# george-gca/sr-pytorch-lightning

Hardware: AMD Instinct MI355X
Metric: SR training throughput, LR patches/s (48x48 LR x4, fwd+bwd+Adam) (higher is better)
Workload: dtype bf16; 1 GPU; edsr_baseline x4, 48x48 LR patches, batch 256/GPU, train step (L1 + Adam); global_batch=256, parallelism=dp1, hip_graph=full

## Files before the change

sr-pytorch-lightning_amd/csrc/conv_lk.hip:

```cpp
#include <stdlib.h>
#include <type_traits>
#include "srk_common.h"

#ifndef SRK_LK5_STAMPS
#define SRK_LK5_STAMPS 0
#endif

namespace {

template <int DT, int CPP, int NRB, int K>
__global__ __launch_bounds__(256) void lk_conv_kernel(const srk_conv_args a, int tilesX, int tilesY, unsigned x_bytes, unsigned w_bytes) {
  typedef DTraits<DT> Tr;
  constexpr int PXB = CPP * 16;
  constexpr int ROWS = 32 * NRB;
  extern __shared__ __attribute__((aligned(16))) char smem[];
  constexpr int XT = 16 + K - 1, XTP = (XT + 1) & ~1;
  constexpr int xs_bytes = XT * XTP * PXB;
  constexpr int slab = K * CPP * ROWS * 16;
  char* const Xs = smem;
  char* const Wr = smem + ((xs_bytes + 1023) & ~1023);

  const int tid = threadIdx.x, lane = tid & 63;
  const int wave = __builtin_amdgcn_readfirstlane(tid >> 6);
  const int r = lane & 31, h = lane >> 5;
// ... 764 lines not shown
    {
      int n, y0, x0;
      tile_of(t, n, y0, x0);
#pragma unroll
      for (int pb = 0; pb < 2; ++pb) {
        const int gy = y0 + prow[pb], gx = x0 + px;
        const bool ok = h == 0 && gy < H && gx < W;
#pragma unroll
        for (int o = 0; o < 4; ++o) {
          if (o >= O) break;
#pragma unroll
          for (int i = 0; i < 2; ++i) {
            typedef __attribute__((ext_vector_type(2))) unsigned int u32x2_t;
            u32x2_t v;
            v.x = __float_as_uint(acc[pb][o * 4 + i * 2] * sc + pa[o]);
            v.y = __float_as_uint(acc[pb][o * 4 + i * 2 + 1] * sc + pa[o]);
            const unsigned off = ok ? (unsigned)((((n * O + o) * H2 + 2 * gy + i) * W2 + 2 * gx) * 4) : 0x80000000u;
            __builtin_amdgcn_raw_buffer_store_b64(v, orsrc, off, 0, SRK_AUX_WT);
          }
        }
      }
    }
  }
}

template <int DT, int NW>
__global__ __launch_bounds__(NW * 64) void lk5_rows_fwd_kernel(const srk_conv_args a, int nb, int segs, int seg_rows, int units, unsigned x_bytes) {
  typedef DTraits<DT> Tr;
  constexpr int AHEAD = NW == 4 ? 2 : 1, PRO = NW + 4 + (AHEAD - 1) * NW, RING = PRO + NW;
  constexpr int ROWB = 32 * 128, SP = 68, SCR = 32 * SP * 4;
  extern __shared__ __attribute__((aligned(16))) char smem[];
  const int tid = threadIdx.x, lane = tid & 63;
  const int wave = __builtin_amdgcn_readfirstlane(tid >> 6);
  const int r = lane & 31, h = lane >> 5;
  const int H = a.H, W = a.W, O = a.Cout >> 2;
  float* const scr = reinterpret_cast<float*>(smem + RING * ROWB + wave * SCR);
  const unsigned lds0 = lds_addr_of(smem);
  const __amdgpu_buffer_rsrc_t wrs = __builtin_amdgcn_make_buffer_rsrc(const_cast<void*>(a.wpk), 0, 25 * 8 * 32 * 16, 0x00020000);
  const i32x4 xrsrc = make_rsrc4(a.x, x_bytes);

  float bias6[6], pa3[3];
#pragma unroll
  for (int o = 0; o < 3; ++o) {
    pa3[o] = (a.post_add && o < O) ? a.post_add[o] : 0.f;
#pragma unroll
    for (int j = 0; j < 2; ++j) bias6[o * 2 + j] = (a.bias && o < O) ? a.bias[8 * o + h * 2 + j] : 0.f;
  }
  typedef __attribute__((ext_vector_type(4))) unsigned int u32x4_t;
  i32x4 A[5][4][2];
#pragma unroll
  for (int m = 0; m < 2; ++m) {
    const int R = m * 32 + r, kw = R / 12, co = R - kw * 12;
    const bool ok = R < 60 && co < a.Cout;
#pragma unroll
    for (int kh = 0; kh < 5; ++kh)
#pragma unroll
      for (int ks = 0; ks < 4; ++ks) {
        const unsigned off = ok ? (unsigned)(((((kh * 5 + kw) * 8 + 2 * ks + h) * 32 + 8 * (co >> 2) + (co & 3)) << 4)) : 0x80000000u;
        const u32x4_t v = __builtin_amdgcn_raw_buffer_load_b128(wrs, off, 0, 0);
        A[kh][ks][m] = i32x4{(int)v.x, (int)v.y, (int)v.z, (int)v.w};
      }
  }
  int ccol[4], cpx[4];
#pragma unroll
  for (int pc = 0; pc < 4; ++pc) {
    const int px = pc * 8 + (lane >> 3), sl = lane & 7, c = sl ^ swz(px);
    cpx[pc] = px - 2;
    ccol[pc] = ((px - 2) * a.x_pitch + a.x_coff + c * 8) * 2;
  }
  asm volatile("s_waitcnt vmcnt(0)" ::: "memory");

  const int bsw = swz(r);
  const int H2 = 2 * H, W2 = 2 * W;
  const float sc = a.scale;
  const __amdgpu_buffer_rsrc_t orsrc = __builtin_amdgcn_make_buffer_rsrc(a.out, 0, 0x7fffffff, 0x00020000);

  for (int u = blockIdx.x; u < units; u += gridDim.x) {
    const int sgm = u % segs, bb = (u / segs) % nb, n = u / (segs * nb);
    const int x0 = bb * 28, ys = sgm * seg_rows;
    const int ye = min(H, ys + seg_rows), nx = min(28, W - x0);
    const int steps = (ye - ys + NW - 1) / NW, qmax = (ye - ys) + 4;
    auto dma_row = [&](int q) {
      const int gy = ys - 2 + q;
      const bool rok = (unsigned)gy < (unsigned)H && q < qmax;
      const int base = ((n * H + gy) * W + x0) * a.x_pitch * 2;
      const unsigned dst = lds0 + (unsigned)((q % RING) * ROWB);
#pragma unroll
      for (int pc = 0; pc < 4; ++pc) {
        const bool ok = rok && (unsigned)(x0 + cpx[pc]) < (unsigned)W;
        dma16_hidden(xrsrc, ok ? (unsigned)(base + ccol[pc]) : 0x80000000u, (unsigned)__builtin_amdgcn_readfirstlane((int)(dst + pc * 1024)));
      }
    };
    asm volatile("s_waitcnt vmcnt(0) lgkmcnt(0)\n\ts_barrier" ::: "memory");
    for (int q = wave; q < PRO; q += NW) dma_row(q);

    f32x16 accp[2];
    int gyp = 0;
    auto epi_write = [&](int g0, int cnt) {
#pragma unroll
      for (int g = g0; g < g0 + cnt; ++g) {
        const int m = g >> 2, i = g & 3;
        *reinterpret_cast<f32x4*>(scr + r * SP + m * 32 + 8 * i + 4 * h) = f32x4{accp[m][4 * i], accp[m][4 * i + 1], accp[m][4 * i + 2], accp[m][4 * i + 3]};
      }
    };
    float ev[6];
    auto epi_read = [&](int t0, int cnt) {
#pragma unroll
      for (int t = t0; t < t0 + cnt; ++t) {
        const int o = t / 5, kw = t - o * 5;
        const f32x2 v = *reinterpret_cast<const f32x2*>(scr + (r + kw) * SP + kw * 12 + o * 4 + h * 2);
        ev[o * 2] = kw == 0 ? v.x : ev[o * 2] + v.x;
        ev[o * 2 + 1] = kw == 0 ? v.y : ev[o * 2 + 1] + v.y;
      }
    };
    auto epi_store = [&]() {
      const bool ok = r < nx && gyp < ye;
#pragma unroll
      for (int o = 0; o < 3; ++o) {
        typedef __attribute__((ext_vector_type(2))) unsigned int u32x2_t;
        u32x2_t v;
        v.x = __float_as_uint((ev[o * 2] + bias6[o * 2]) * sc + pa3[o]);
        v.y = __float_as_uint((ev[o * 2 + 1] + bias6[o * 2 + 1]) * sc + pa3[o]);
        const unsigned off = (ok && o < O) ? (unsigned)((((n * O + o) * H2 + 2 * gyp + h) * W2 + 2 * (x0 + r)) * 4) : 0x80000000u;
        __builtin_amdgcn_raw_buffer_store_b64(v, orsrc, off, 0, SRK_AUX_WT);
      }
    };
    auto step = [&](int s, auto epi_tag) {
      constexpr bool EPI = decltype(epi_tag)::value;
      if (!EPI) asm volatile("s_waitcnt vmcnt(0)" ::: "memory");
      else if (AHEAD == 1) { if (s == 1) asm volatile("s_waitcnt vmcnt(0)" ::: "memory"); else asm volatile("s_waitcnt vmcnt(3)" ::: "memory"); }
      else if (s == 1) asm volatile("s_waitcnt vmcnt(4)" ::: "memory");
      else if (s == 2) asm volatile("s_waitcnt vmcnt(7)" ::: "memory");
      else asm volatile("s_waitcnt vmcnt(10)" ::: "memory");
      asm volatile("s_waitcnt lgkmcnt(0)\n\ts_barrier" ::: "memory");
      dma_row(NW * s + PRO + wave);
      const int q0 = NW * s + wave;
      const char* rowp[5];
#pragma unroll
      for (int kh = 0; kh < 5; ++kh) rowp[kh] = smem + ((q0 + kh) % RING) * ROWB + r * 128;
      f32x16 acc[2];
#pragma unroll
      for (int e = 0; e < 16; ++e) { acc[0][e] = 0.f; acc[1][e] = 0.f; }
      constexpr int PF = 6;
      i32x4 bf[PF];
      auto bfrag = [&](int k) { return lds_read16(rowp[k >> 2] + (((2 * (k & 3) + h) ^ bsw) << 4)); };
#pragma unroll
      for (int k = 0; k < PF; ++k) bf[k] = bfrag(k);
#pragma unroll
      for (int k = 0; k < 20; ++k) {
        const i32x4 b = bf[k % PF];
        if (k + PF < 20) bf[k % PF] = bfrag(k + PF);
        if (EPI) {
          if (k < 8) epi_write(k, 1);
          else if (k == 8) asm volatile("" ::: "memory");
          else if (k >= 9 && k < 19) epi_read((k - 9) * 3 / 2, (k - 8) * 3 / 2 - (k - 9) * 3 / 2);
          else if (k == 19) epi_store();
        }
        acc[0] = Tr::mma(A[k >> 2][k & 3][0], b, acc[0]);
        acc[1] = Tr::mma(A[k >> 2][k & 3][1], b, acc[1]);
        __builtin_amdgcn_sched_barrier(0);
      }
      accp[0] = acc[0]; accp[1] = acc[1];
      gyp = ys + q0;
    };
    step(0, std::false_type{});
#pragma unroll 1
    for (int s = 1; s < steps; ++s) step(s, std::true_type{});
    epi_write(0, 8);
    asm volatile("" ::: "memory");
    epi_read(0, 15);
    epi_store();
  }
}

template <int DT>
__global__ __launch_bounds__(256) void lk5_dgrad_kernel(const srk_conv_args a, int nb, int segs, int seg_rows, int units, unsigned x_bytes) {
  typedef DTraits<DT> Tr;
  typedef typename Tr::elem elem;
  constexpr int RING = 16, ROWB = 36 * 32;
  extern __shared__ __attribute__((aligned(16))) char smem[];
  const int tid = threadIdx.x, lane = tid & 63;
  const int wave = __builtin_amdgcn_readfirstlane(tid >> 6);
  const int r = lane & 31, h = lane >> 5;
  const int H = a.H, W = a.W;
  const unsigned lds0 = lds_addr_of(smem);
  const __amdgpu_buffer_rsrc_t wrs = __builtin_amdgcn_make_buffer_rsrc(const_cast<void*>(a.wpk), 0, 25 * 2 * 64 * 16, 0x00020000);
  const i32x4 xrsrc = make_rsrc4(a.x, x_bytes);
  typedef __attribute__((ext_vector_type(4))) unsigned int u32x4_t;
  i32x4 A[25][2];
#pragma unroll
  for (int t = 0; t < 25; ++t)
#pragma unroll
    for (int m = 0; m < 2; ++m) {
      const u32x4_t v = __builtin_amdgcn_raw_buffer_load_b128(wrs, (unsigned)((((t * 2 + h) * 64 + m * 32 + r) << 4)), 0, 0);
      A[t][m] = i32x4{(int)v.x, (int)v.y, (int)v.z, (int)v.w};
    }
  const int c0 = ((lane >> 1) - 2) * a.x_pitch * 2 + (a.x_coff + (lane & 1) * 8) * 2, p0 = (lane >> 1) - 2;
  const int c1 = ((32 + (lane >> 1)) - 2) * a.x_pitch * 2 + (a.x_coff + (lane & 1) * 8) * 2, p1 = 32 + (lane >> 1) - 2;
  asm volatile("s_waitcnt vmcnt(0)" ::: "memory");

  const __amdgpu_buffer_rsrc_t orsrc = __builtin_amdgcn_make_buffer_rsrc(a.out, 0, 0x7fffffff, 0x00020000);
  for (int u = blockIdx.x; u < units; u += gridDim.x) {
    const int sgm = u % segs, bb = (u / segs) % nb, n = u / (segs * nb);
    const int x0 = bb * 32, ys = sgm * seg_rows;
    const int ye = min(H, ys + seg_rows);
    const int steps = (ye - ys + 3) >> 2, qmax = (ye - ys) + 4;
    auto dma_row = [&](int q) {
      const int gy = ys - 2 + q;
      const bool rok = (unsigned)gy < (unsigned)H && q < qmax;
      const int base = ((n * H + gy) * W + x0) * a.x_pitch * 2;
      const unsigned dst = lds0 + (unsigned)((q % RING) * ROWB);
      dma16_hidden(xrsrc, (rok && (unsigned)(x0 + p0) < (unsigned)W) ? (unsigned)(base + c0) : 0x80000000u, (unsigned)__builtin_amdgcn_readfirstlane((int)dst));
      if (lane < 8)
        dma16_hidden(xrsrc, (rok && (unsigned)(x0 + p1) < (unsigned)W) ? (unsigned)(base + c1) : 0x80000000u, (unsigned)__builtin_amdgcn_readfirstlane((int)(dst + 1024)));
    };
    asm volatile("s_waitcnt vmcnt(0) lgkmcnt(0)\n\ts_barrier" ::: "memory");
    dma_row(wave);
    dma_row(4 + wave);
    dma_row(8 + wave);
#if SRK_LK5_STAMPS
    unsigned long long* const stamp = (blockIdx.x == 0 && tid == 0 && u == blockIdx.x) ? reinterpret_cast<unsigned long long*>(const_cast<float*>(a.post_add)) : nullptr;
#define SRK_LSTAMP(i) do { if (stamp && s < 24) stamp[s * 8 + (i)] = __builtin_amdgcn_s_memtime(); } while (0)
#else
#define SRK_LSTAMP(i) do { } while (0)
#endif
    f32x16 accp[2];
    int gyp = 0;
    uint32_t P[4][4];
    auto epi_cvt = [&](int k) {
#pragma unroll
      for (int d = 0; d < 4; ++d) P[k][d] = pack2<DT>(accp[k >> 1][8 * (k & 1) + 2 * d], accp[k >> 1][8 * (k & 1) + 2 * d + 1]);
    };
    auto epi_store = [&](int j) {
      const int qi = r & 3, gxq = x0 + (r & ~3);
      const bool ok = gyp < ye && gxq + j < W;
      const unsigned off = (unsigned)((((n * H + gyp) * W + gxq + j) * a.out_pitch + a.out_coff + 32 * h + 8 * qi) * 2);
      const u32x4_t ov = {P[j][0], P[j][1], P[j][2], P[j][3]};
      __builtin_amdgcn_raw_buffer_store_b128(ov, orsrc, ok ? off : 0x80000000u, 0, SRK_AUX_WT);
    };
    auto step = [&](int s, auto epi_tag) {
      constexpr bool EPI = decltype(epi_tag)::value;
      SRK_LSTAMP(0);
      if (!EPI) asm volatile("s_waitcnt vmcnt(0)" ::: "memory");
      else if (s == 1) asm volatile("s_waitcnt vmcnt(2)" ::: "memory");
      else if (s == 2) asm volatile("s_waitcnt vmcnt(6)" ::: "memory");
      else asm volatile("s_waitcnt vmcnt(10)" ::: "memory");
      SRK_LSTAMP(1);
      asm volatile("s_waitcnt lgkmcnt(0)\n\ts_barrier" ::: "memory");
      SRK_LSTAMP(2);
      dma_row(4 * s + 12 + wave);
      const int q0 = 4 * s + wave;
      const char* rowp[5];
#pragma unroll
      for (int kh = 0; kh < 5; ++kh) rowp[kh] = smem + ((q0 + kh) % RING) * ROWB + r * 32 + h * 16;
      f32x16 acc[2];
#pragma unroll
      for (int e = 0; e < 16; ++e) { acc[0][e] = 0.f; acc[1][e] = 0.f; }
      constexpr int PF = 6;
      i32x4 bf[PF];
      auto bfrag = [&](int t) { return lds_read16(rowp[t / 5] + (t % 5) * 32); };
#pragma unroll
      for (int t = 0; t < PF; ++t) bf[t] = bfrag(t);
#pragma unroll
      for (int t = 0; t < 25; t += 2) {
        const i32x4 b0 = bf[t % PF], b1 = bf[(t + 1) % PF];
        if (t + PF < 25) bf[t % PF] = bfrag(t + PF);
        if (t + 1 + PF < 25) bf[(t + 1) % PF] = bfrag(t + 1 + PF);
        if (EPI) {
          if (t >= 2 && t < 10) epi_cvt((t - 2) >> 1);
          else if (t == 10) quad_transpose8_dpp(P[0][0], P[1][0], P[2][0], P[3][0], P[0][1], P[1][1], P[2][1], P[3][1]);
          else if (t == 12) quad_transpose8_dpp(P[0][2], P[1][2], P[2][2], P[3][2], P[0][3], P[1][3], P[2][3], P[3][3]);
          else if (t >= 14 && t < 22) epi_store((t - 14) >> 1);
        }
        acc[0] = Tr::mma(A[t][0], b0, acc[0]);
        if (t + 1 < 25) acc[0] = Tr::mma(A[t + 1][0], b1, acc[0]);
        acc[1] = Tr::mma(A[t][1], b0, acc[1]);
        if (t + 1 < 25) acc[1] = Tr::mma(A[t + 1][1], b1, acc[1]);
        __builtin_amdgcn_sched_barrier(0);
      }
      SRK_LSTAMP(3);
      accp[0] = acc[0]; accp[1] = acc[1];
      gyp = ys + q0;
    };
    step(0, std::false_type{});
#pragma unroll 1
    for (int s = 1; s < steps; ++s) step(s, std::true_type{});
#pragma unroll
    for (int k = 0; k < 4; ++k) epi_cvt(k);
    quad_transpose8_dpp(P[0][0], P[1][0], P[2][0], P[3][0], P[0][1], P[1][1], P[2][1], P[3][1]);
    quad_transpose8_dpp(P[0][2], P[1][2], P[2][2], P[3][2], P[0][3], P[1][3], P[2][3], P[3][3]);
#pragma unroll
    for (int j = 0; j < 4; ++j) epi_store(j);
  }
}

SRK_DEV void lk5_pair(int t, int& fyA, int& fxA, int& fyB, int& fxB, bool& hasB) {
  hasB = true;
  if (t < 5) { fyA = -2; fxA = t - 2; fyB = -1; fxB = t - 2; }
  else if (t < 10) { fyA = 0; fxA = t - 7; fyB = 1; fxB = t - 7; }
  else if (t == 10) { fyA = 2; fxA = -2; fyB = 2; fxB = 2; }
  else { fyA = 2; fxA = t - 12; fyB = 2; fxB = t - 12; hasB = false; }
}

template <int DT>
__global__ __launch_bounds__(256) void lk5_wgrad_kernel(const srk_wgrad_args a, int tilesX, int tilesY, int tq, int trem,
                                                        unsigned x_bytes, unsigned dy_bytes) {
  typedef DTraits<DT> Tr;
  constexpr int XB = 16 * 16 * 128, DP = 20, DB = 13 * 1024, BUF = XB + DB;
  extern __shared__ __attribute__((aligned(16))) char smem[];
  const int tid = threadIdx.x, lane = tid & 63;
  const int wave = __builtin_amdgcn_readfirstlane(tid >> 6);
  const int slot = blockIdx.x;
  const int H = a.H, W = a.W;
  const int t0 = slot * tq + min(slot, trem), nt = tq + (slot < trem ? 1 : 0);
  const i32x4 xrs = make_rsrc4(a.x, x_bytes), drs = make_rsrc4(a.dy, dy_bytes);
  const unsigned lds0 = lds_addr_of(smem);

  int xconst[8], xyx[8];
#pragma unroll
  for (int k = 0; k < 8; ++k) {
    const int i = tid + 256 * k, sl = i & 7, p = i >> 3, iy = p >> 4, ix = p & 15, c = sl ^ swz(ix);
    xconst[k] = ((iy * W + ix) * a.x_pitch + a.x_coff + c * 8) * 2;
    xyx[k] = iy | (ix << 8);
  }
  int dconst[4], dyx[4];
#pragma unroll
  for (int j = 0; j < 4; ++j) {
    const int i = tid + 256 * j, c = i & 1, pp = i >> 1, iy = pp / DP, ix = pp - iy * DP;
    dconst[j] = (((iy - 2) * W + (ix - 2)) * a.dy_pitch + a.dy_coff + c * 8) * 2;
    dyx[j] = i < 2 * DP * DP ? (((iy - 2) & 0xffff) | ((ix - 2) << 16)) : (int)0x7fff7fff;
  }
  auto dma_tile = [&](int tile, int b) {
    int pt = tile;
    const int tX = pt % tilesX;
    pt /= tilesX;
    const int tY = pt % tilesY;
    const int n = pt / tilesY;
    const int y0 = tY * 16, x0 = tX * 16;
    const int xbase = ((n * H + y0) * W + x0) * a.x_pitch * 2, dbase = ((n * H + y0) * W + x0) * a.dy_pitch * 2;
#pragma unroll
    for (int k = 0; k < 8; ++k) {
      const bool ok = y0 + (xyx[k] & 255) < H && x0 + (xyx[k] >> 8) < W;
      dma16_hidden(xrs, ok ? (unsigned)(xbase + xconst[k]) : 0x80000000u,
                   (unsigned)__builtin_amdgcn_readfirstlane((int)(lds0 + b * BUF + ((k * 256 + wave * 64) << 4))));
    }
#pragma unroll
    for (int j = 0; j < 4; ++j) {
      if (j * 256 + wave * 64 >= 2 * DP * DP) continue;
      const int gy = y0 + (int)(short)(dyx[j] & 0xffff), gx = x0 + (dyx[j] >> 16);
      const bool ok = (unsigned)gy < (unsigned)H && (unsigned)gx < (unsigned)W;
      dma16_hidden(drs, ok ? (unsigned)(dbase + dconst[j]) : 0x80000000u,
                   (unsigned)__builtin_amdgcn_readfirstlane((int)(lds0 + b * BUF + XB + ((j * 256 + wave * 64) << 4))));
    }
  };

  const int rb = wave & 1, half = wave >> 1;
  f32x16 acc[7];
#pragma unroll
  for (int j = 0; j < 7; ++j)
#pragma unroll
    for (int e = 0; e < 16; ++e) acc[j][e] = 0.f;
  int aoff[2], boff[7][2];
#pragma unroll
  for (int rd = 0; rd < 2; ++rd) aoff[rd] = tr_lane_off(0, rd, rb, lane);
  {
    const int G = lane >> 4, q = (lane & 15) >> 2, pq = lane & 3;
#pragma unroll
    for (int j = 0; j < 7; ++j) {
      int fyA, fxA, fyB, fxB; bool hasB;
      lk5_pair(half * 7 + j, fyA, fxA, fyB, fxB, hasB);
      const int fy = (G & 1) ? fyB : fyA, fx = (G & 1) ? fxB : fxA;
#pragma unroll
      for (int rd = 0; rd < 2; ++rd) {
        const int col = 8 * (G >> 1) + 4 * rd + q;
        boff[j][rd] = ((2 - fy) * DP + (col - fx + 2)) * 32 + pq * 8;
      }
    }
  }
  const bool do_bias = a.dbp != nullptr && wave == 2;
  float dbz = 0.f;

  const int pieces_of = 8 + (wave == 0 ? 4 : 3);
  if (nt > 0) dma_tile(t0, 0);
  if (nt > 1) dma_tile(t0 + 1, 1);
#if SRK_LK5_STAMPS
  unsigned long long* const wstamp = (blockIdx.x == 0 && tid == 0 && a.dbp) ? reinterpret_cast<unsigned long long*>(a.dbp) + (size_t)a.nslabs * 8 : nullptr;
#define SRK_WSTAMP(i) do { if (wstamp && it < 24) wstamp[it * 8 + (i)] = __builtin_amdgcn_s_memtime(); } while (0)
#else
#define SRK_WSTAMP(i) do { } while (0)
#endif
  for (int it = 0; it < nt; ++it) {
    SRK_WSTAMP(0);
    const char* const X = smem + (it % 3) * BUF;
    const char* const D = X + XB;
    if (it + 1 < nt) { if (pieces_of == 12) asm volatile("s_waitcnt vmcnt(12)" ::: "memory"); else asm volatile("s_waitcnt vmcnt(11)" ::: "memory"); }
    else asm volatile("s_waitcnt vmcnt(0)" ::: "memory");
    SRK_WSTAMP(1);
    asm volatile("s_waitcnt lgkmcnt(0)\n\ts_barrier" ::: "memory");
    SRK_WSTAMP(2);
    if (it + 2 < nt) dma_tile(t0 + it + 2, (it + 2) % 3);
    SRK_WSTAMP(3);
    i32x4 afn, bfn[7];
    auto fetch = [&](int y) {
      afn = tr_read2(X + y * 2048 + aoff[0], X + y * 2048 + aoff[1]);
#pragma unroll
      for (int j = 0; j < 7; ++j) bfn[j] = tr_read2(D + y * (DP * 32) + boff[j][0], D + y * (DP * 32) + boff[j][1]);
    };
    fetch(0);
#pragma unroll 2
    for (int y = 0; y < 16; ++y) {
      const i32x4 af = afn;
      i32x4 bf[7];
#pragma unroll
      for (int j = 0; j < 7; ++j) bf[j] = bfn[j];
      if (y + 1 < 16) fetch(y + 1);
      if (do_bias) {
        const int qw[4] = {bf[0].x, bf[0].y, bf[0].z, bf[0].w};
#pragma unroll
        for (int e = 0; e < 4; ++e) {
          float f0, f1;
          unpack2<DT>((uint32_t)qw[e], f0, f1);
          dbz += f0 + f1;
        }
      }
#pragma unroll
      for (int j = 0; j < 7; ++j) acc[j] = Tr::mma(af, bf[j], acc[j]);
    }
    SRK_WSTAMP(4);
  }

  if (do_bias) {
    dbz += __shfl_xor(dbz, 32, 64);
    if (lane < 16) a.dbp[(size_t)slot * 16 + lane] = dbz;
  }
  {
    const int hq = lane >> 5, n = lane & 31, co = n & 15;
    float* const sl = a.dwp + (size_t)slot * (25 * 64 * 16);
#pragma unroll
    for (int j = 0; j < 7; ++j) {
      int fyA, fxA, fyB, fxB; bool hasB;
      lk5_pair(half * 7 + j, fyA, fxA, fyB, fxB, hasB);
      if (n >= 16 && !hasB) continue;
      const int tap = n < 16 ? (fyA + 2) * 5 + fxA + 2 : (fyB + 2) * 5 + fxB + 2;
#pragma unroll
      for (int e = 0; e < 16; ++e) {
        const int ci = rb * 32 + 4 * hq + (e & 3) + 8 * (e >> 2);
        sl[((size_t)tap * 64 + ci) * 16 + co] = acc[j][e];
      }
    }
  }
}

bool lk5_wgrad_ok(const srk_wgrad_args& a) {
  static const bool off = [] { const char* e = srk_dbg_getenv("SRK_NO_LK5"); return e && e[0] == '1'; }();
  return !off && a.KH == 5 && a.Cin == 64 && a.Cout == 16 && (a.cout_real == 0 || a.cout_real > 6) && a.x_pitch % 8 == 0 && a.dy_pitch % 8 == 0 &&
         a.x_coff % 8 == 0 && a.dy_coff % 8 == 0;
}

bool lk_all_rows(const srk_wgrad_args& a) {
  static const bool off = [] { const char* e = srk_dbg_getenv("SRK_NO_LK_ALLROWS"); const char* p = srk_dbg_getenv("SRK_NO_LK_PACKED"); return (e && e[0] == '1') || (p && p[0] == '1'); }();
  return !off && a.cout_real > 0 && a.cout_real <= LK_CS && a.cout_real * a.KW <= 32 && a.KH >= 5;
}

int lk_wgrad_slabs_for(const srk_wgrad_args& a) {
  static const int cus = [] { int c = srk_device_cus(); return c > 0 ? c : 256; }();
  if (lk_all_rows(a)) {
    const long long nt8 = (long long)a.N * ((a.H + LK_TR - 1) / LK_TR) * ((a.W + 15) / 16);
    return (int)(nt8 < cus ? nt8 : cus);
  }
  const long long ntiles = (long long)a.N * ((a.H + 15) / 16) * ((a.W + 15) / 16);
  if (lk5_wgrad_ok(a)) return (int)(ntiles < cus ? ntiles : cus);
  long long s = cus / a.KH;
  if (s < 1) s = 1;
  if (s > ntiles) s = ntiles;
  return (int)s;
}

}

bool srk_conv_lk_ok(const srk_conv_args& a) {
  if (a.dtype == SRK_F32 || a.KH != a.KW || a.KH < 5 || a.KH > 9 || !(a.KH & 1)) return false;
  if (a.x_ps > 1 || a.mask) return false;
  const bool fwd = a.Cin == 64 && a.CoutP == 32;
  const bool bwd = a.Cin == 16 && a.CoutP == 64;
  if (!fwd && !bwd) return false;
  if (a.out_mode == SRK_OUT_PLANAR) {
    if (!fwd || a.ps_r != 2 || a.res || a.relu || a.Cout % 4 || a.Cout > 16 || a.x_pitch % 8 || a.x_coff % 8) return false;
    return (long long)a.N * a.H * a.W * a.x_pitch * 2 < 0x7fff0000LL;
  }
  if (a.out_mode != SRK_OUT_NHWC || (a.post_add && !SRK_LK5_STAMPS)) return false;
  if (a.x_pitch % 8 || a.x_coff % 8 || a.out_pitch % 8 || a.out_coff % 8 || a.Cout % 8 || (a.res && (a.res_pitch % 8 || a.res_coff % 8))) return false;
  const long long px = (long long)a.N * a.H * a.W;
  long long mx = px * a.x_pitch;
  if (px * a.out_pitch > mx) mx = px * a.out_pitch;
  return mx * 2 < 0x7fff0000LL;
}

template <int DT, int CPP, int NRB, int K> static int lk_launch_k(const srk_conv_args& a, hipStream_t st) {
  constexpr int XT = 16 + K - 1, XTP = (XT + 1) & ~1;
  constexpr int xs = (XT * XTP * CPP * 16 + 1023) & ~1023, slab = K * CPP * 32 * NRB * 16;
  constexpr int lds = xs + 2 * slab;
  static const hipError_t attr = hipFuncSetAttribute(reinterpret_cast<const void*>(&lk_conv_kernel<DT, CPP, NRB, K>),
                                                     hipFuncAttributeMaxDynamicSharedMemorySize, 160 * 1024);
  if (attr != hipSuccess) { srk_set_error("srk_conv2d: cannot reserve LDS for the large-kernel conv"); return (int)attr; }
  SRK_CHECK_ARG(lds <= 160 * 1024, "srk_conv2d: %dx%d kernel needs %d bytes of LDS", K, K, lds);
  const int tilesX = (a.W + 15) / 16, tilesY = (a.H + 15) / 16;
  const long long nb = (long long)a.N * tilesX * tilesY;
  SRK_CHECK_ARG(nb <= 0x7fffffffLL, "srk_conv2d: %lld workgroups", nb);
  hipLaunchKernelGGL((lk_conv_kernel<DT, CPP, NRB, K>), dim3((unsigned)nb), dim3(256), lds, st, a, tilesX, tilesY,
                     (unsigned)((long long)a.N * a.H * a.W * a.x_pitch * 2), (unsigned)((long long)K * slab));
  SRK_LAUNCH_CHECK();
  return 0;
}
template <int DT, int CPP, int NRB> static int lk_launch(const srk_conv_args& a, hipStream_t st) {
  switch (a.KH) {
    case 5: return lk_launch_k<DT, CPP, NRB, 5>(a, st);
    case 7: return lk_launch_k<DT, CPP, NRB, 7>(a, st);
    default: return lk_launch_k<DT, CPP, NRB, 9>(a, st);
  }
}

template <int DT, int K> static int lk_rows_launch_k(const srk_conv_args& a, hipStream_t st) {
  constexpr int XWP = (16 + K - 1 + 1) & ~1, XR = 8 + K - 1;
  constexpr int lds = ((XR * XWP * 128 + 1023) & ~1023) + 4 * 4096 + 4 * 512;
  static_assert(lds <= 80 * 1024, "two workgroups per CU");
  static const hipError_t attr = hipFuncSetAttribute(reinterpret_cast<const void*>(&lk_conv_rows_kernel<DT, K>), hipFuncAttributeMaxDynamicSharedMemorySize, lds);
  if (attr != hipSuccess) { srk_set_error("srk_conv2d: cannot reserve LDS for the large-kernel conv"); return (int)attr; }
  const int tilesX = (a.W + 15) / 16, tilesY = (a.H + 7) / 8;
  const long long nb = (long long)a.N * tilesX * tilesY;
  SRK_CHECK_ARG(nb <= 0x7fffffffLL, "srk_conv2d: %lld workgroups", nb);
  hipLaunchKernelGGL((lk_conv_rows_kernel<DT, K>), dim3((unsigned)nb), dim3(256), lds, st, a, tilesX, tilesY,
                     (unsigned)((long long)a.N * a.H * a.W * a.x_pitch * 2), (unsigned)((long long)K * K * 64 * a.CoutP * 2));
  SRK_LAUNCH_CHECK();
  return 0;
}
template <int DT> static int lk_rows_launch(const srk_conv_args& a, hipStream_t st) {
  switch (a.KH) {
    case 5: return lk_rows_launch_k<DT, 5>(a, st);
    case 7: return lk_rows_launch_k<DT, 7>(a, st);
    default: return lk_rows_launch_k<DT, 9>(a, st);
  }
}

template <int DT, int NW> static int lk5_rows_fwd_launch_w(const srk_conv_args& a, hipStream_t st) {
  constexpr int PRO = NW + 4 + (NW == 4 ? NW : 0), lds = (PRO + NW) * 32 * 128 + NW * 32 * 68 * 4;
  static const int cus = [] { int c = srk_device_cus(); return c > 0 ? c : 256; }();
  static const hipError_t attr = hipFuncSetAttribute(reinterpret_cast<const void*>(&lk5_rows_fwd_kernel<DT, NW>), hipFuncAttributeMaxDynamicSharedMemorySize, lds);
  if (attr != hipSuccess) { srk_set_error("srk_conv2d: cannot reserve LDS for the 5x5 image conv"); return (int)attr; }
  const int nb = (a.W + 27) / 28;
  int segs = (int)(cus / ((long long)a.N * nb));
  const int max_segs = (a.H + 7) / 8;
  if (segs > max_segs) segs = max_segs;
  if (segs < 1) segs = 1;
  const int seg_rows = (((a.H + segs - 1) / segs) + NW - 1) / NW * NW;
  segs = (a.H + seg_rows - 1) / seg_rows;
  const long long units = (long long)a.N * nb * segs;
  SRK_CHECK_ARG(units <= 0x7fffffffLL, "srk_conv2d: %lld units", units);
  const int grid = (int)(units < cus ? units : cus);
  hipLaunchKernelGGL((lk5_rows_fwd_kernel<DT, NW>), dim3(grid), dim3(NW * 64), lds, st, a, nb, segs, seg_rows, (int)units,
                     (unsigned)((long long)a.N * a.H * a.W * a.x_pitch * 2));
  SRK_LAUNCH_CHECK();
  return 0;
}
template <int DT> static int lk5_rows_fwd_launch(const srk_conv_args& a, hipStream_t st) { return lk5_rows_fwd_launch_w<DT, 4>(a, st); }

static bool lk5_dgrad_ok(const srk_conv_args& a) {
  return a.KH == 5 && a.Cin == 16 && a.CoutP == 64 && a.Cout == 64 && a.out_mode == SRK_OUT_NHWC && !a.bias && !a.res && !a.relu && !a.mask &&
         (SRK_LK5_STAMPS || !a.post_add) && a.scale == 1.f && (long long)a.N * a.H * a.W * a.out_pitch * 2 < 0x7fff0000LL;
}
template <int DT> static int lk5_dgrad_launch(const srk_conv_args& a, hipStream_t st) {
  constexpr int lds = 16 * 36 * 32;
  static const int cus = [] { int c = srk_device_cus(); return c > 0 ? c : 256; }();
  const int nb = (a.W + 31) / 32;
  int segs = (int)(cus / ((long long)a.N * nb));
  const int max_segs = (a.H + 7) / 8;
  if (segs > max_segs) segs = max_segs;
  if (segs < 1) segs = 1;
  const int seg_rows = (((a.H + segs - 1) / segs) + 3) & ~3;
  segs = (a.H + seg_rows - 1) / seg_rows;
  const long long units = (long long)a.N * nb * segs;
  SRK_CHECK_ARG(units <= 0x7fffffffLL, "srk_conv2d: %lld units", units);
  const int grid = (int)(units < cus ? units : cus);
  hipLaunchKernelGGL((lk5_dgrad_kernel<DT>), dim3(grid), dim3(256), lds, st, a, nb, segs, seg_rows, (int)units,
                     (unsigned)((long long)a.N * a.H * a.W * a.x_pitch * 2));
  SRK_LAUNCH_CHECK();
  return 0;
}

template <int DT> static int lk5_fwd_launch(const srk_conv_args& a, hipStream_t st) {
  constexpr int lds = 25 * 8 * 16 * 16 + 2 * 20 * 20 * 128;
  static const int cus = [] { int c = srk_device_cus(); return c > 0 ? c : 256; }();
  static const hipError_t attr = hipFuncSetAttribute(reinterpret_cast<const void*>(&lk5_fwd_kernel<DT>), hipFuncAttributeMaxDynamicSharedMemorySize, 160 * 1024);
  if (attr != hipSuccess) { srk_set_error("srk_conv2d: cannot reserve LDS for the 5x5 image conv"); return (int)attr; }
  const int tilesX = (a.W + 15) / 16, tilesY = (a.H + 15) / 16;
  const long long ntiles = (long long)a.N * tilesX * tilesY;
  SRK_CHECK_ARG(ntiles <= 0x7fffffffLL, "srk_conv2d: %lld tiles", ntiles);
  const int slots = (int)(ntiles < cus ? ntiles : cus);
  hipLaunchKernelGGL((lk5_fwd_kernel<DT>), dim3(slots), dim3(256), lds, st, a, tilesX, tilesY, (int)(ntiles / slots), (int)(ntiles % slots),
                     (unsigned)((long long)a.N * a.H * a.W * a.x_pitch * 2));
  SRK_LAUNCH_CHECK();
  return 0;
}

int srk_conv_lk_launch(const srk_conv_args& a, hipStream_t st) {
  static const bool no_lk5 = [] { const char* e = srk_dbg_getenv("SRK_NO_LK5"); return e && e[0] == '1'; }();
  static const bool no_lk5_rows = [] { const char* e = srk_dbg_getenv("SRK_NO_LK5_ROWS"); return e && e[0] == '1'; }();
  if (a.out_mode == SRK_OUT_PLANAR && a.KH == 5 && !no_lk5 && !no_lk5_rows && a.Cout <= 12)
    return a.dtype == SRK_BF16 ? lk5_rows_fwd_launch<SRK_BF16>(a, st) : lk5_rows_fwd_launch<SRK_F16>(a, st);
  if (a.out_mode == SRK_OUT_PLANAR && a.KH == 5 && !no_lk5) return a.dtype == SRK_BF16 ? lk5_fwd_launch<SRK_BF16>(a, st) : lk5_fwd_launch<SRK_F16>(a, st);
  static const bool no_rows = [] { const char* e = srk_dbg_getenv("SRK_NO_LK_ROWS"); return e && e[0] == '1'; }();
  if (!no_rows && a.out_mode == SRK_OUT_NHWC && a.Cin == 64 && a.cout_real > 0 && a.cout_real <= 4 && a.cout_real * a.KW <= 32 && a.Cout == 16 && !a.relu && !a.res && a.scale == 1.f)
    return a.dtype == SRK_BF16 ? lk_rows_launch<SRK_BF16>(a, st) : lk_rows_launch<SRK_F16>(a, st);
  static const bool no_lk5_dgrad = [] { const char* e = srk_dbg_getenv("SRK_NO_LK5_DGRAD"); return e && e[0] == '1'; }();
  if (!no_lk5 && !no_lk5_dgrad && lk5_dgrad_ok(a)) return a.dtype == SRK_BF16 ? lk5_dgrad_launch<SRK_BF16>(a, st) : lk5_dgrad_launch<SRK_F16>(a, st);
  if (a.Cin == 16) return a.dtype == SRK_BF16 ? lk_launch<SRK_BF16, 2, 2>(a, st) : lk_launch<SRK_F16, 2, 2>(a, st);
  return a.dtype == SRK_BF16 ? lk_launch<SRK_BF16, 8, 1>(a, st) : lk_launch<SRK_F16, 8, 1>(a, st);
}

bool srk_wgrad_lk_ok(const srk_wgrad_args& a) {
  if (a.dtype == SRK_F32 || a.KH != a.KW || a.KH < 5 || a.KH > 9 || !(a.KH & 1)) return false;
  if (a.x_ps > 1 || a.dy_ps > 1 || a.Cin > 64 || a.Cin % 16 || a.Cout > 32 || a.Cout % 8) return false;
  const long long px = (long long)a.N * a.H * a.W;
  return px * a.x_pitch * 2 < 0x7fff0000LL && px * a.dy_pitch * 2 < 0x7fff0000LL;
}
int srk_wgrad_lk_slabs(const srk_wgrad_args& a) { return lk_wgrad_slabs_for(a); }
int srk_wgrad_lk_slab_cout(const srk_wgrad_args& a) { return lk_all_rows(a) ? LK_CS : a.Cout; }

template <int DT, int K> static int lk_wgrad_launch_k(const srk_wgrad_args& a, hipStream_t st) {
  constexpr int XWP = (16 + K - 1 + 1) & ~1;
  constexpr int lds = 2 * (16 * XWP * 128 + 16 * 16 * 32 + 1024);
  static const hipError_t attr = hipFuncSetAttribute(reinterpret_cast<const void*>(&lk_wgrad_kernel<DT, K>), hipFuncAttributeMaxDynamicSharedMemorySize, 160 * 1024);
  if (attr != hipSuccess) { srk_set_error("srk_conv2d_wgrad: cannot reserve LDS"); return (int)attr; }
  const int tilesX = (a.W + 15) / 16, tilesY = (a.H + 15) / 16;
  const long long ntiles = (long long)a.N * tilesX * tilesY;
  const int slabs = a.nslabs;
  const unsigned xb = (unsigned)((long long)a.N * a.H * a.W * a.x_pitch * 2), db = (unsigned)((long long)a.N * a.H * a.W * a.dy_pitch * 2);
  if (lk_all_rows(a)) {
    constexpr int XR = LK_TR + K - 1;
    constexpr int alds = 2 * (((XR * XWP * 128 + 1023) & ~1023) + LK_TR * 16 * 32) + 8 * LK_TR * (16 + 2 * (K - 1) + 16) * 2;
    static_assert(alds <= 160 * 1024, "LDS");
    static const hipError_t aattr = hipFuncSetAttribute(reinterpret_cast<const void*>(&lk_wgrad_allrows_kernel<DT, K>), hipFuncAttributeMaxDynamicSharedMemorySize, 160 * 1024);
    if (aattr != hipSuccess) { srk_set_error("srk_conv2d_wgrad: cannot reserve LDS"); return (int)aattr; }
    const int tY8 = (a.H + LK_TR - 1) / LK_TR;
    const long long nt8 = (long long)a.N * tY8 * tilesX;
    hipLaunchKernelGGL((lk_wgrad_allrows_kernel<DT, K>), dim3(slabs), dim3(256), alds, st, a, tilesX, tY8, (int)nt8, (int)(nt8 / slabs), (int)(nt8 % slabs), xb, db);
    SRK_LAUNCH_CHECK();
    return 0;
  }
  if constexpr (K == 5) {
    if (lk5_wgrad_ok(a)) {
      constexpr int l5 = 3 * (16 * 16 * 128 + 13 * 1024);
      static const hipError_t a5 = hipFuncSetAttribute(reinterpret_cast<const void*>(&lk5_wgrad_kernel<DT>), hipFuncAttributeMaxDynamicSharedMemorySize, 160 * 1024);
      if (a5 != hipSuccess) { srk_set_error("srk_conv2d_wgrad: cannot reserve LDS"); return (int)a5; }
      hipLaunchKernelGGL((lk5_wgrad_kernel<DT>), dim3(slabs), dim3(256), l5, st, a, tilesX, tilesY, (int)(ntiles / slabs), (int)(ntiles % slabs), xb, db);
      SRK_LAUNCH_CHECK();
      return 0;
    }
  }
  static const bool no_packed = [] { const char* e = srk_dbg_getenv("SRK_NO_LK_PACKED"); return e && e[0] == '1'; }();
  if (a.cout_real > 0 && a.cout_real <= 6 && a.cout_real * K <= 32 && !no_packed) {
    constexpr int plds = 2 * (16 * XWP * 128 + 16 * 16 * 32) + 8 * 16 * (16 + 2 * (K - 1) + 16) * 2 + 2 * 16 * 64 * 4;
    static_assert(plds <= 160 * 1024, "LDS");
    static const hipError_t pattr = hipFuncSetAttribute(reinterpret_cast<const void*>(&lk_wgrad_packed_kernel<DT, K>), hipFuncAttributeMaxDynamicSharedMemorySize, 160 * 1024);
    if (pattr != hipSuccess) { srk_set_error("srk_conv2d_wgrad: cannot reserve LDS"); return (int)pattr; }
    hipLaunchKernelGGL((lk_wgrad_packed_kernel<DT, K>), dim3(slabs, K), dim3(256), plds, st, a, tilesX, tilesY, (int)ntiles, (int)(ntiles / slabs), (int)(ntiles % slabs), xb, db);
    SRK_LAUNCH_CHECK();
    return 0;
  }
  hipLaunchKernelGGL((lk_wgrad_kernel<DT, K>), dim3(slabs, K), dim3(256), lds, st, a, tilesX, tilesY, (int)ntiles, (int)(ntiles / slabs), (int)(ntiles % slabs), xb, db);
  SRK_LAUNCH_CHECK();
  return 0;
}
template <int DT> static int lk_wgrad_launch_dt(const srk_wgrad_args& a, hipStream_t st) {
  switch (a.KH) {
    case 5: return lk_wgrad_launch_k<DT, 5>(a, st);
    case 7: return lk_wgrad_launch_k<DT, 7>(a, st);
    default: return lk_wgrad_launch_k<DT, 9>(a, st);
  }
}
int srk_wgrad_lk_launch(const srk_wgrad_args& a, hipStream_t st) {
  return a.dtype == SRK_BF16 ? lk_wgrad_launch_dt<SRK_BF16>(a, st) : lk_wgrad_launch_dt<SRK_F16>(a, st);
}
```

Baseline: 46540 LR patches/s.

## Reuse dy fragments across vertical tap pairs and interleave DMA in lk5 wgrad

```diff
diff --git a/sr-pytorch-lightning_amd/csrc/conv_lk.hip b/sr-pytorch-lightning_amd/csrc/conv_lk.hip
--- a/sr-pytorch-lightning_amd/csrc/conv_lk.hip
+++ b/sr-pytorch-lightning_amd/csrc/conv_lk.hip
@@ -1090,6 +1090,12 @@
   else { fyA = 2; fxA = t - 12; fyB = 2; fxB = t - 12; hasB = false; }
 }
 
+constexpr int lk5_reused(int half) { return half == 0 ? 3 : 2; }
+constexpr int lk5_deal(int half, int j) {
+  return half == 0 ? (j < 6 ? (j >> 1) + 5 * (j & 1) : 10)
+                   : (j < 4 ? 3 + (j >> 1) + 5 * (j & 1) : 7 + j);
+}
+
 template <int DT>
 __global__ __launch_bounds__(256) void lk5_wgrad_kernel(const srk_wgrad_args a, int tilesX, int tilesY, int tq, int trem,
                                                         unsigned x_bytes, unsigned dy_bytes) {
@@ -1118,28 +1124,35 @@
     dconst[j] = (((iy - 2) * W + (ix - 2)) * a.dy_pitch + a.dy_coff + c * 8) * 2;
     dyx[j] = i < 2 * DP * DP ? (((iy - 2) & 0xffff) | ((ix - 2) << 16)) : (int)0x7fff7fff;
   }
-  auto dma_tile = [&](int tile, int b) {
+  struct TileAt { int y0, x0, xbase, dbase; };
+  auto tile_at = [&](int tile) {
     int pt = tile;
     const int tX = pt % tilesX;
     pt /= tilesX;
     const int tY = pt % tilesY;
     const int n = pt / tilesY;
     const int y0 = tY * 16, x0 = tX * 16;
-    const int xbase = ((n * H + y0) * W + x0) * a.x_pitch * 2, dbase = ((n * H + y0) * W + x0) * a.dy_pitch * 2;
-#pragma unroll
-    for (int k = 0; k < 8; ++k) {
-      const bool ok = y0 + (xyx[k] & 255) < H && x0 + (xyx[k] >> 8) < W;
-      dma16_hidden(xrs, ok ? (unsigned)(xbase + xconst[k]) : 0x80000000u,
+    return TileAt{y0, x0, ((n * H + y0) * W + x0) * a.x_pitch * 2, ((n * H + y0) * W + x0) * a.dy_pitch * 2};
+  };
+  auto dma_piece = [&](const TileAt& t, int b, int p) {
+    if (p < 8) {
+      const int k = p;
+      const bool ok = t.y0 + (xyx[k] & 255) < H && t.x0 + (xyx[k] >> 8) < W;
+      dma16_hidden(xrs, ok ? (unsigned)(t.xbase + xconst[k]) : 0x80000000u,
                    (unsigned)__builtin_amdgcn_readfirstlane((int)(lds0 + b * BUF + ((k * 256 + wave * 64) << 4))));
-    }
-#pragma unroll
-    for (int j = 0; j < 4; ++j) {
-      if (j * 256 + wave * 64 >= 2 * DP * DP) continue;
-      const int gy = y0 + (int)(short)(dyx[j] & 0xffff), gx = x0 + (dyx[j] >> 16);
+    } else {
+      const int j = p - 8;
+      if (j * 256 + wave * 64 >= 2 * DP * DP) return;
+      const int gy = t.y0 + (int)(short)(dyx[j] & 0xffff), gx = t.x0 + (dyx[j] >> 16);
       const bool ok = (unsigned)gy < (unsigned)H && (unsigned)gx < (unsigned)W;
-      dma16_hidden(drs, ok ? (unsigned)(dbase + dconst[j]) : 0x80000000u,
+      dma16_hidden(drs, ok ? (unsigned)(t.dbase + dconst[j]) : 0x80000000u,
                    (unsigned)__builtin_amdgcn_readfirstlane((int)(lds0 + b * BUF + XB + ((j * 256 + wave * 64) << 4))));
     }
+  };
+  auto dma_tile = [&](int tile, int b) {
+    const TileAt t = tile_at(tile);
+#pragma unroll
+    for (int p = 0; p < 12; ++p) dma_piece(t, b, p);
   };
 
   const int rb = wave & 1, half = wave >> 1;
@@ -1148,24 +1161,10 @@
   for (int j = 0; j < 7; ++j)
 #pragma unroll
     for (int e = 0; e < 16; ++e) acc[j][e] = 0.f;
-  int aoff[2], boff[7][2];
+  int aoff[2];
 #pragma unroll
   for (int rd = 0; rd < 2; ++rd) aoff[rd] = tr_lane_off(0, rd, rb, lane);
-  {
-    const int G = lane >> 4, q = (lane & 15) >> 2, pq = lane & 3;
-#pragma unroll
-    for (int j = 0; j < 7; ++j) {
-      int fyA, fxA, fyB, fxB; bool hasB;
-      lk5_pair(half * 7 + j, fyA, fxA, fyB, fxB, hasB);
-      const int fy = (G & 1) ? fyB : fyA, fx = (G & 1) ? fxB : fxA;
-#pragma unroll
-      for (int rd = 0; rd < 2; ++rd) {
-        const int col = 8 * (G >> 1) + 4 * rd + q;
-        boff[j][rd] = ((2 - fy) * DP + (col - fx + 2)) * 32 + pq * 8;
-      }
-    }
-  }
-  const bool do_bias = a.dbp != nullptr && wave == 2;
+  const bool do_bias = a.dbp != nullptr && wave == 0;
   float dbz = 0.f;
 
   const int pieces_of = 8 + (wave == 0 ? 4 : 3);
@@ -1177,45 +1176,94 @@
 #else
 #define SRK_WSTAMP(i) do { } while (0)
 #endif
-  for (int it = 0; it < nt; ++it) {
-    SRK_WSTAMP(0);
-    const char* const X = smem + (it % 3) * BUF;
-    const char* const D = X + XB;
-    if (it + 1 < nt) { if (pieces_of == 12) asm volatile("s_waitcnt vmcnt(12)" ::: "memory"); else asm volatile("s_waitcnt vmcnt(11)" ::: "memory"); }
-    else asm volatile("s_waitcnt vmcnt(0)" ::: "memory");
-    SRK_WSTAMP(1);
-    asm volatile("s_waitcnt lgkmcnt(0)\n\ts_barrier" ::: "memory");
-    SRK_WSTAMP(2);
-    if (it + 2 < nt) dma_tile(t0 + it + 2, (it + 2) % 3);
-    SRK_WSTAMP(3);
-    i32x4 afn, bfn[7];
-    auto fetch = [&](int y) {
-      afn = tr_read2(X + y * 2048 + aoff[0], X + y * 2048 + aoff[1]);
-#pragma unroll
-      for (int j = 0; j < 7; ++j) bfn[j] = tr_read2(D + y * (DP * 32) + boff[j][0], D + y * (DP * 32) + boff[j][1]);
-    };
-    fetch(0);
-#pragma unroll 2
-    for (int y = 0; y < 16; ++y) {
-      const i32x4 af = afn;
-      i32x4 bf[7];
-#pragma unroll
-      for (int j = 0; j < 7; ++j) bf[j] = bfn[j];
-      if (y + 1 < 16) fetch(y + 1);
-      if (do_bias) {
-        const int qw[4] = {bf[0].x, bf[0].y, bf[0].z, bf[0].w};
-#pragma unroll
-        for (int e = 0; e < 4; ++e) {
+  auto tiles = [&](auto HC, auto BC) {
+    constexpr int HALF = decltype(HC)::value, NR = lk5_reused(HALF), NL = 7 - 2 * NR, NG = 1 + NR + NL;
+    constexpr bool BIAS = decltype(BC)::value;
+    int boff[NR + NL];
+    {
+      const int G = lane >> 4, q = (lane & 15) >> 2, pq = lane & 3;
+#pragma unroll
+      for (int k = 0; k < NR + NL; ++k) {
+        int fyA, fxA, fyB, fxB; bool hasB;
+        lk5_pair(lk5_deal(HALF, k < NR ? 2 * k : NR + k), fyA, fxA, fyB, fxB, hasB);
+        const int fy = (G & 1) ? fyB : fyA, fx = (G & 1) ? fxB : fxA;
+        boff[k] = ((2 - fy) * DP + (8 * (G >> 1) + q - fx + 2)) * 32 + pq * 8;
+      }
+    }
+    for (int it = 0; it < nt; ++it) {
+      SRK_WSTAMP(0);
+      if (it + 1 < nt) { if (pieces_of == 12) asm volatile("s_waitcnt vmcnt(12)" ::: "memory"); else asm volatile("s_waitcnt vmcnt(11)" ::: "memory"); }
+      else asm volatile("s_waitcnt vmcnt(0)" ::: "memory");
+      SRK_WSTAMP(1);
+      asm volatile("s_waitcnt lgkmcnt(0)\n\ts_barrier" ::: "memory");
+      SRK_WSTAMP(2);
+      const bool more = it + 2 < nt;
+      const TileAt nx = tile_at(more ? t0 + it + 2 : t0);
+      const int nb = (it + 2) % 3;
+      SRK_WSTAMP(3);
+      i32x4 xf[2], fr[NR][3], fl[NL][2];
+      unsigned xa[2], fa[NR + NL];
+#pragma unroll
+      for (int rd = 0; rd < 2; ++rd) { xa[rd] = lds0 + (unsigned)((it % 3) * BUF + aoff[rd]); asm volatile("" : "+v"(xa[rd])); }
+#pragma unroll
+      for (int k = 0; k < NR + NL; ++k) {
+        fa[k] = lds0 + (unsigned)((it % 3) * BUF + XB + boff[k] - (k < NR ? 2 * DP * 32 : 0));
+        asm volatile("" : "+v"(fa[k]));
+      }
+      auto lds_tr2 = [](unsigned a0, unsigned a1) {
+        typedef __attribute__((address_space(3))) i16x4 lds_i16x4;
+        const i16x4 lo = __builtin_amdgcn_ds_read_tr16_b64_v4i16((lds_i16x4*)(size_t)a0);
+        const i16x4 hi = __builtin_amdgcn_ds_read_tr16_b64_v4i16((lds_i16x4*)(size_t)a1);
+        const i32x2 l2 = __builtin_bit_cast(i32x2, lo), h2 = __builtin_bit_cast(i32x2, hi);
+        return i32x4{l2.x, l2.y, h2.x, h2.y};
+      };
+      auto read_x = [&](int y) { xf[y & 1] = lds_tr2(xa[0] + y * 2048, xa[1] + y * 2048); };
+      auto read_r = [&](int k, int y) { fr[k][(y + 3) % 3] = lds_tr2(fa[k] + (y + 2) * (DP * 32), fa[k] + (y + 2) * (DP * 32) + 128); };
+      auto read_l = [&](int m, int y) { fl[m][y & 1] = lds_tr2(fa[NR + m] + y * (DP * 32), fa[NR + m] + y * (DP * 32) + 128); };
+      auto read_group = [&](int g, int y) {
+        if (g == 0) read_x(y);
+        else if (g <= NR) read_r(g - 1, y);
+        else read_l(g - 1 - NR, y);
+      };
+      auto bias_word = [&](int r, int e) {
+        if constexpr (BIAS) {
+          const i32x4 b7 = fr[2][(r + 1) % 3];
+          const int qw[4] = {b7.x, b7.y, b7.z, b7.w};
           float f0, f1;
           unpack2<DT>((uint32_t)qw[e], f0, f1);
-          dbz += f0 + f1;
+          float t;
+          asm("v_add_f32 %0, %1, %2" : "=v"(t) : "v"(f0), "v"(f1));
+          dbz += t;
         }
-      }
-#pragma unroll
-      for (int j = 0; j < 7; ++j) acc[j] = Tr::mma(af, bf[j], acc[j]);
-    }
-    SRK_WSTAMP(4);
-  }
+      };
+#pragma unroll
+      for (int k = 0; k < NR; ++k) { read_r(k, -2); read_r(k, -1); }
+#pragma unroll
+      for (int g = 0; g < NG; ++g) read_group(g, 0);
+#pragma unroll
+      for (int y = 0; y < 16; ++y) {
+        const i32x4 af = xf[y & 1];
+        __builtin_amdgcn_sched_barrier(0);
+#pragma unroll
+        for (int i = 0; i < 7; ++i) {
+          if (i < NR) acc[2 * i + 1] = Tr::mma(af, fr[i][(y + 1) % 3], acc[2 * i + 1]);
+          else if (i < 2 * NR) acc[2 * (i - NR)] = Tr::mma(af, fr[i - NR][y % 3], acc[2 * (i - NR)]);
+          else acc[i] = Tr::mma(af, fl[i - 2 * NR][y & 1], acc[i]);
+          if (BIAS) {
+            if (y == 0) { if (i < 2) { bias_word(0, 2 * i); bias_word(0, 2 * i + 1); } else if (i < 6) bias_word(1, i - 2); }
+            else if (y < 15 && i < 4) bias_word(y + 1, i);
+          }
+          if (i < NG && y + 1 < 16) read_group(i, y + 1);
+          if (i == 6 && y < 12 && more) dma_piece(nx, nb, y);
+          __builtin_amdgcn_sched_barrier(0);
+        }
+      }
+      SRK_WSTAMP(4);
+    }
+  };
+  if (do_bias) tiles(std::integral_constant<int, 0>{}, std::true_type{});
+  else if (half == 0) tiles(std::integral_constant<int, 0>{}, std::false_type{});
+  else tiles(std::integral_constant<int, 1>{}, std::false_type{});
 
   if (do_bias) {
     dbz += __shfl_xor(dbz, 32, 64);
@@ -1227,7 +1275,7 @@
 #pragma unroll
     for (int j = 0; j < 7; ++j) {
       int fyA, fxA, fyB, fxB; bool hasB;
-      lk5_pair(half * 7 + j, fyA, fxA, fyB, fxB, hasB);
+      lk5_pair(lk5_deal(half, j), fyA, fxA, fyB, fxB, hasB);
       if (n >= 16 && !hasB) continue;
       const int tap = n < 16 ? (fyA + 2) * 5 + fxA + 2 : (fyB + 2) * 5 + fxB + 2;
 #pragma unroll
```

Result: faster. 47020 LR patches/s, median of 6 (+1.0%).
